# nemjit001/surf-path-tracer

Measured on AMD Instinct MI355X. Metric: Mrays/s at 1280×720, 256 spp, indoor scene; 1/2/4/8 MI355X + CPU ref, higher is better.
Workload: dtype f32; 1 GPU; C3; scene=bundled indoor (main.cpp:161-346), width=1280, height=720, spp=256, renders=7, step=one complete 256-frame render including its drain, bounces=unbounded + russian roulette, zero_cutoff=True, parallelism=single GPU

## Files before the change

surf-path-tracer_amd/csrc/device/types.h:

```cpp
#pragma once
#include <hip/hip_runtime.h>
#include <stdint.h>
#include "lds_layout.h"

namespace surfdev {

constexpr uint32_t kUnset = 0xffffffffu;
constexpr uint32_t kFlagMedium = 1u, kFlagSpecular = 2u;
constexpr int kBlock = 256;

struct DevInstance {
    float Minv[16];
    float M[16];
    uint32_t triOffset, idxOffset, nodeOffset, material;
    float area;
    uint32_t affineInv;
    uint32_t affine;
    uint32_t _pad;
};

struct DevMaterial {
    float emit, refl, refr, ior;
    float ec[4], albedo[4], absorb[4];
};

struct TraceInst {
    float4 m0, m1, m2, m3;
    uint4 meta;
    float4 r0, r1, r2, r3;
    float4 wlo, whi;
};
constexpr uint32_t kLdsTraceInst = 64;

struct DevScene {
    const TraceInst* tinst;
    const float4* nodes;
    const float4* tris;
    const float4* normals;
    const float4* verts;
    const float4* tlasNodes;
    const uint32_t* tlasIdx;
    const DevInstance* inst;
    const DevMaterial* mats;
    const uint2* lights;
    uint32_t nLights;
    uint32_t sbNode0, sbRecN, sbTri0, sbTriN;
    const float4* sbRec;
    uint32_t nInst, nMats;
    uint32_t tlasLeafCount;
    uint32_t finiteBoxes;
    uint32_t nodes4G;
    const float* wnodes;
    uint32_t nWnodes;
    uint32_t laneW;
    uint32_t bgType;
    float bgColor[3], bgA[3], bgB[3];
    float cellLo[3], cellScale[3];
    uint32_t nHeavy, keyMode;
    float4 hvLo[3], hvHi[3];
};

struct DevCamera {
    float pos[3], firstPixel[3], uVec[3], vVec[3], diskU[3], diskV[3];
    float invW, invH;
    uint32_t defocus;
};

struct Pool { float4* od; float4* T; uint8_t* key; };

constexpr uint32_t kShBins = 16;
#ifndef SURF_SH_XCDS
#define SURF_SH_XCDS 1
#endif
#ifndef SURF_SH_STRIDE
#define SURF_SH_STRIDE 32
#endif
constexpr uint32_t kShXcds = SURF_SH_XCDS, kShStride = SURF_SH_STRIDE;
constexpr uint32_t kShSegs = kShBins * kShXcds + 1u;
struct ShadowQ {
    float4* od; float4* c;
    uint32_t* cur;
    uint32_t region;
    uint32_t bins;
};

struct Counters {
    uint32_t nIn[2];
    uint32_t app[2];
    uint32_t maxSeg;
    uint32_t zeroCutoff;
    uint32_t segMax;
    uint32_t survN;
    uint32_t survCap;
    uint32_t rowNext;
    uint32_t permFrames, permA;
    uint32_t spp;
    unsigned long long issued[2];
    unsigned long long limit;
    unsigned long long baseFrame;
    unsigned long long ev[16];
    uint32_t capped[64];
    unsigned long long evS[32][16];
    unsigned long long dbg[8];
};
constexpr uint32_t kStripes = 32;
constexpr int kEvents = 9;

struct StreamGeom {
    const uint32_t* rows;
    uint32_t width, npx, window;
    const uint32_t* perm;
};

constexpr uint32_t kLeafTagC = 0x80000000u;
constexpr uint32_t kLeafTag = 0x80000000u;
constexpr uint32_t kLeafInW = 3;

constexpr uint32_t kLdsInst = 64, kLdsMats = 64, kLdsLights = 64;

constexpr int kDenoiseMaxIterations = 6;

static_assert(sizeof(TraceInst) == 4 * layout::kTraceInstWords && sizeof(DevInstance) == 4 * layout::kInstanceWords &&
                  sizeof(DevMaterial) == 4 * layout::kMaterialWords && sizeof(uint2) == 4 * layout::kLightWords &&
                  sizeof(float4) * 4 == 4 * layout::kNodeRecWords && sizeof(float4) * 3 == 4 * layout::kTriRecWords,
              "lds_layout.h states the table elements' sizes");

}
```

surf-path-tracer_amd/csrc/device/wavefront_kernels.h:

```cpp
#pragma once
#include <hip/hip_runtime.h>
#include <type_traits>
#include "surf_math.h"
#include "types.h"

namespace surfdev {

#ifndef SURF_SHADE_WAVES
#define SURF_SHADE_WAVES 4
#endif
#ifndef SURF_SEG_TIMING
#define SURF_SEG_TIMING 0
#endif
#ifndef SURF_TAIL_WAVES
#define SURF_TAIL_WAVES 3
#endif
#ifndef SURF_TRACE_WAVES
#define SURF_TRACE_WAVES 2
#endif
#ifndef SURF_TRACE_WAVES_EXT
#define SURF_TRACE_WAVES_EXT 6
#endif
#ifndef SURF_COOP_WAVES
#define SURF_COOP_WAVES 4
// ... 268 lines not shown
                    } else {
                        float eL, eR;
                        wBoxes<FIN>(rc, o, rd, depth, eL, eR);
                        bool g;
                        if (ANY) g = eL == kFarAway;
                        else g = eL > eR;
                        const float en = g ? eR : eL, ef = g ? eL : eR;
                        if (en == kFarAway) {
                            if (df == kFarAway) goto pop;
                            ref = refF;
                            continue;
                        }
                        if (df != kFarAway) { *sp = refF; sp += stride; }
                        const uint32_t pN = f2u(g ? rc.d.w : rc.d.z), pF = f2u(g ? rc.d.z : rc.d.w);
                        if (ef != kFarAway) { *sp = pF ? pF : nodeOff + lC + (g ? 0u : 1u); sp += stride; }
                        ref = pN ? pN : nodeOff + lC + (g ? 1u : 0u);
                        continue;
                    }
                }
            }
        }
        if (leafTest<ANY>(tri, lf, cnt, o, d, depth, hu, hv, hprim)) {
            if (ANY) return true;
            any = true;
        }
    pop:
        if (sp == bottom) break;
        sp -= stride;
        ref = *sp;
    }
    return any;
}

__device__ __forceinline__ float rowDot(float4 r, float x, float y, float z, float w) {
    const float a = r.x * x + r.y * y;
    const float b = r.z * z + r.w * w;
    return a + b;
}

__device__ __forceinline__ void instanceRay(const TraceInst& I, V3 o, V3 d, V3& oo, V3& dd) {
    oo = mk3(rowDot(I.m0, o.x, o.y, o.z, 1.0f), rowDot(I.m1, o.x, o.y, o.z, 1.0f), rowDot(I.m2, o.x, o.y, o.z, 1.0f));
    if (!I.meta.z) oo = divs(oo, rowDot(I.m3, o.x, o.y, o.z, 1.0f));
    dd = mk3(rowDot(I.m0, d.x, d.y, d.z, 0.0f), rowDot(I.m1, d.x, d.y, d.z, 0.0f), rowDot(I.m2, d.x, d.y, d.z, 0.0f));
}

template <bool ANY, bool LW = false, bool STG = false, typename SK = uint32_t>
__device__ __forceinline__ bool instanceTrace(const DevScene& S, const TraceInst& I, V3 o, V3 d, float& depth, float& hu,
                                              float& hv, uint32_t& hprim, SK* stk, uint32_t stride, uint32_t base,
                                              const float4* sN = nullptr) {
    V3 oo, dd;
    instanceRay(I, o, d, oo, dd);
    if (f2u(I.r1.w) != 0u)
        return leafTestUniform<ANY>(S.tris + 3u * I.meta.y, f2u(I.r0.w), f2u(I.r1.w), oo, dd, depth, hu, hv, hprim);
    const V3 rd = mk3(1.0f / dd.x, 1.0f / dd.y, 1.0f / dd.z);
    const bool fin = S.finiteBoxes && finite3(oo) && finite3(rd);
    if constexpr (LW)
        return fin ? blasTraceW<ANY, true>(S, I, oo, dd, rd, depth, hu, hv, hprim, stk, stride, base)
                   : blasTraceW<ANY, false>(S, I, oo, dd, rd, depth, hu, hv, hprim, stk, stride, base);
    if (fin) return blasTrace<ANY, true, STG, SK>(S, I, oo, dd, rd, depth, hu, hv, hprim, stk, stride, base, sN);
    return blasTrace<ANY, false, STG, SK>(S, I, oo, dd, rd, depth, hu, hv, hprim, stk, stride, base, sN);
}

struct TraceTables {
    const TraceInst* inst;
    const uint32_t* order;
};

__device__ __forceinline__ TraceTables stageTrace(const DevScene& S, uint32_t* lds, uint32_t at) {
    TraceInst* tab = reinterpret_cast<TraceInst*>(lds + at);
    uint32_t* order = reinterpret_cast<uint32_t*>(tab + S.nInst);
    const uint32_t n16 = S.nInst * (uint32_t)(sizeof(TraceInst) / 16);
    for (uint32_t k = threadIdx.x; k < n16; k += blockDim.x) reinterpret_cast<float4*>(tab)[k] = reinterpret_cast<const float4*>(S.tinst)[k];
    for (uint32_t k = threadIdx.x; k < S.nInst; k += blockDim.x) order[k] = S.tlasIdx[k];
    __syncthreads();
    return TraceTables{tab, order};
}

template <bool LDS_INST>
__device__ __forceinline__ TraceTables traceTables(const DevScene& S, uint32_t* lds, uint32_t at) {
    if (LDS_INST) return stageTrace(S, lds, at);
    return TraceTables{S.tinst, S.tlasIdx};
}

template <bool ANY, bool LW = false, bool STG = false, typename SK = uint32_t>
__device__ __forceinline__ bool traceScene(const DevScene& S, const TraceTables& Tt, V3 o, V3 d, float& depth, float& hu, float& hv,
                                           uint32_t& hinst, uint32_t& hprim, SK* stk, uint32_t stride, const float4* sN = nullptr) {
    bool any = false;
    if (S.tlasLeafCount) {
        const V3 rdw = mk3(1.0f / d.x, 1.0f / d.y, 1.0f / d.z);
        const bool cullOk = finite3(o) && finite3(rdw);
        for (uint32_t k = 0; k < S.tlasLeafCount; ++k) {
            const uint32_t ii = Tt.order[k];
            const TraceInst& I = Tt.inst[ii];
            if (cullOk && I.wlo.w != 0.0f) {
                const float tx0 = (I.wlo.x - o.x) * rdw.x, tx1 = (I.whi.x - o.x) * rdw.x;
                const float ty0 = (I.wlo.y - o.y) * rdw.y, ty1 = (I.whi.y - o.y) * rdw.y;
                const float tz0 = (I.wlo.z - o.z) * rdw.z, tz1 = (I.whi.z - o.z) * rdw.z;
                const float t0 = fmaxf(fmaxf(fminf(tx0, tx1), fminf(ty0, ty1)), fminf(tz0, tz1));
                const float t1 = fminf(fminf(fmaxf(tx0, tx1), fmaxf(ty0, ty1)), fmaxf(tz0, tz1));
                if (t1 < t0 || t1 < 0.0f || t0 >= depth) continue;
            }
            const bool hitI = (STG && !LW && I.meta.x == S.sbNode0 && I.meta.y == S.sbTri0)
                                  ? instanceTrace<ANY, false, true, SK>(S, I, o, d, depth, hu, hv, hprim, stk, stride, 0u, sN)
                                  : instanceTrace<ANY, LW, false, SK>(S, I, o, d, depth, hu, hv, hprim, stk, stride, 0u);
            if (hitI) {
                if (ANY) return true;
                any = true;
                hinst = ii;
            }
        }
        return any;
    }
    const V3 rd = mk3(1.0f / d.x, 1.0f / d.y, 1.0f / d.z);
    uint32_t sp = 0, node = 0;
    for (;;) {
        const float4* nd = S.tlasNodes + 4u * node;
        float4 q0 = nd[0], q1 = nd[1], q2 = nd[2], q3 = nd[3];
        pin(q0); pin(q1); pin(q2); pin(q3);
        const uint32_t lf = f2u(q0.w), cnt = f2u(q1.w);
        if (cnt != 0u) {
            for (uint32_t k = 0; k < cnt; ++k) {
                const uint32_t ii = Tt.order[lf + k];
                if (instanceTrace<ANY, LW, false, SK>(S, Tt.inst[ii], o, d, depth, hu, hv, hprim, stk, stride, sp)) {
                    if (ANY) return true;
                    any = true;
                    hinst = ii;
                }
            }
            if (sp == 0) break;
            node = stk[(--sp) * stride];
            continue;
        }
        float dn = slab(q0.x, q0.y, q0.z, q1.x, q1.y, q1.z, o, rd, depth);
        float df = slab(q2.x, q2.y, q2.z, q3.x, q3.y, q3.z, o, rd, depth);
        uint32_t cn = lf, cf = lf + 1u;
        if (dn > df) { const float t = dn; dn = df; df = t; const uint32_t c = cn; cn = cf; cf = c; }
        if (dn == kFarAway) {
            if (sp == 0) break;
            node = stk[(--sp) * stride];
        } else {
            node = cn;
            if (df != kFarAway) stk[(sp++) * stride] = cf;
        }
    }
    return any;
}

template <int CTRL>
__device__ __forceinline__ float dppMov(float v) {
    return __int_as_float(__builtin_amdgcn_mov_dpp(__float_as_int(v), CTRL, 0xF, 0xF, false));
}
constexpr int kDppSwap1 = 0xB1;
constexpr int kDppShr2 = 0x112, kDppShr4 = 0x114;

__device__ __forceinline__ uint32_t planeDword(uint32_t l) {
    if (l < 12u) return (l / 6u) * 8u + (l & 1u) * 4u + ((l % 6u) >> 1);
    return l == 12u ? 3u : (l == 13u ? 7u : 0u);
}
__device__ __forceinline__ float pick3(V3 v, uint32_t a) { return a == 0u ? v.x : (a == 1u ? v.y : v.z); }

__device__ __forceinline__ void slabPair(float v, float oA, float rdA, float depth, float& d0, float& d1) {
    const float t = (v - oA) * rdA;
    const float tp = dppMov<kDppSwap1>(t);
    const float t0a = tmin(t, tp), t1a = tmax(t, tp);
    const float t0x = dppMov<kDppShr4>(t0a), t0y = dppMov<kDppShr2>(t0a);
    const float t1x = dppMov<kDppShr4>(t1a), t1y = dppMov<kDppShr2>(t1a);
    const float m0 = tmax(tmax(t0x, t0y), t0a);
    const float m1 = tmin(tmin(t1x, t1y), t1a);
    const float dist = (m1 >= m0 && m0 < depth && m1 > 0.0f) ? m0 : kFarAway;
    d0 = __int_as_float(__builtin_amdgcn_readlane(__float_as_int(dist), 4));
    d1 = __int_as_float(__builtin_amdgcn_readlane(__float_as_int(dist), 10));
}

template <bool ANY>
// ... 2181 lines not shown
```

surf-path-tracer_amd/csrc/host/scene_upload.hip:

```cpp
#include "host/surf_ctx.h"

#include <algorithm>
#include <cfloat>
#include <cmath>
#include <cstdlib>
#include <cstring>

#include "device/surf_math.h"

namespace {

struct TreeWalk {
    uint32_t depth = 0;
    bool ok = true;
    std::string why;
};

TreeWalk walkTree(const surf_bvh_node* nodes, uint32_t nodeCount, uint32_t offset, uint32_t idxCount, uint32_t idxOffset,
                  std::vector<float4>& out, std::vector<uint8_t>& leafSeen, std::vector<uint32_t>* owner = nullptr) {
    TreeWalk w;
    std::vector<std::pair<uint32_t, uint32_t>> st{{0u, 0u}};
    size_t visits = 0;
    while (!st.empty()) {
        auto [local, dep] = st.back();
        st.pop_back();
        if (++visits > (size_t)nodeCount + 1 || dep > 4096) { w.ok = false; w.why = "BVH has a cycle"; return w; }
        const uint64_t g = (uint64_t)offset + local;
        if (g >= nodeCount) { w.ok = false; w.why = "BVH node index out of range"; return w; }
        const surf_bvh_node& n = nodes[g];
        float4* rec = &out[4 * g];
        if (owner) (*owner)[g] = offset;
        rec[0].w = u2f(n.left_first);
        rec[1].w = u2f(n.count);
        if (n.count != 0) {
            if ((uint64_t)idxOffset + n.left_first + n.count > idxCount) { w.ok = false; w.why = "BVH leaf range out of range"; return w; }
            for (uint32_t k = 0; k < n.count; ++k) leafSeen[idxOffset + n.left_first + k] = 1;
            w.depth = std::max(w.depth, dep);
            continue;
        }
        const uint64_t l = (uint64_t)offset + n.left_first;
        if (l + 1 >= nodeCount) { w.ok = false; w.why = "BVH child index out of range"; return w; }
        const surf_bvh_node& L = nodes[l];
        const surf_bvh_node& R = nodes[l + 1];
        rec[0] = make_float4(L.bb_min.x, L.bb_min.y, L.bb_min.z, rec[0].w);
        rec[1] = make_float4(L.bb_max.x, L.bb_max.y, L.bb_max.z, rec[1].w);
        rec[2] = make_float4(R.bb_min.x, R.bb_min.y, R.bb_min.z, 0.0f);
        rec[3] = make_float4(R.bb_max.x, R.bb_max.y, R.bb_max.z, 0.0f);
        st.push_back({n.left_first + 1, dep + 1});
        st.push_back({n.left_first, dep + 1});
    }
    return w;
}

constexpr uint64_t kLdsLightBlas = 20480;

struct InstanceTables {
    std::vector<DevInstance> inst;
    std::vector<TraceInst> tinst;
    std::vector<float4> tnodes;
    std::vector<uint32_t> tidx;
    std::vector<uint2> lights;
    uint32_t tlasDepth = 0, tlasLeafCount = 0;
    uint32_t nHeavy = 0;
    float4 hvLo[3], hvHi[3];
    uint32_t hvInst[3] = {0, 0, 0};
};

void setKeys(surf_ctx* c, DevScene& S, const InstanceTables& T) {
    c->heavyInst.assign(T.hvInst, T.hvInst + T.nHeavy);
    c->permValid = false;
    c->aovValid = false;
    S.nHeavy = T.nHeavy;
    for (uint32_t h = 0; h < 3; ++h) {
        S.hvLo[h] = h < T.nHeavy ? T.hvLo[h] : make_float4(0, 0, 0, 0);
        S.hvHi[h] = h < T.nHeavy ? T.hvHi[h] : make_float4(0, 0, 0, 0);
    }
    S.keyMode = T.nHeavy ? c->keyMode : 0u;
    S.sbNode0 = S.sbRecN = S.sbTri0 = S.sbTriN = 0u;
    S.sbRec = nullptr;
    if (c->ldsLightBlas && !T.lights.empty()) {
        bool one = true;
        const DevInstance* L0 = T.lights[0].x < T.inst.size() ? &T.inst[T.lights[0].x] : nullptr;
        for (const uint2& L : T.lights)
            one = one && L0 && L.x < T.inst.size() && T.inst[L.x].nodeOffset == L0->nodeOffset &&
                  T.inst[L.x].idxOffset == L0->idxOffset && T.inst[L.x].triOffset == L0->triOffset;
        const auto sb = one ? c->stagedBlas.find(L0->nodeOffset) : c->stagedBlas.end();
        const bool small = c->nBlasNodes < 65536u && T.tnodes.size() / 4 < 65536u;
        if (small && sb != c->stagedBlas.end() && sb->second.tri0 == L0->idxOffset) {
            S.sbNode0 = sb->first; S.sbRec = sb->second.rec; S.sbRecN = sb->second.recN;
            S.sbTri0 = sb->second.tri0; S.sbTriN = sb->second.triN;
        }
    }
}

int buildInstanceTables(surf_ctx* c, const surf_gpu_instance* instances, uint32_t n, const uint32_t* tlasIdx,
                        const surf_bvh_node* tlasNodes, uint32_t nTlas, const surf_light* lights, uint32_t nLights, InstanceTables& T) {
    auto affine = [](const float* m) { return m[3] == 0.0f && m[7] == 0.0f && m[11] == 0.0f && m[15] == 1.0f; };
    T.inst.resize(n);
    T.tinst.resize(n);
    for (uint32_t i = 0; i < n; ++i) {
        const surf_gpu_instance& g = instances[i];
        const auto root = c->blasRoots.find(std::make_tuple(g.bvh_node_offset, g.bvh_idx_offset, g.tri_offset));
        if (root == c->blasRoots.end() || g.material_offset >= c->nMaterials)
            return fail(c, SURF_ERR_INVALID, "instance " + std::to_string(i) + ": offsets do not name an uploaded BLAS/material");
        DevInstance& D = T.inst[i];
        std::memcpy(D.Minv, g.inv_transform, sizeof D.Minv);
        std::memcpy(D.M, g.transform, sizeof D.M);
        D.triOffset = g.tri_offset; D.idxOffset = g.bvh_idx_offset; D.nodeOffset = g.bvh_node_offset; D.material = g.material_offset;
        D.area = g.area;
        D.affineInv = affine(g.inv_transform) ? 1u : 0u;
        D.affine = affine(g.transform) ? 1u : 0u;
        const float* m = D.Minv;
        TraceInst& R = T.tinst[i];
        R.m0 = make_float4(m[0], m[4], m[8], m[12]);
        R.m1 = make_float4(m[1], m[5], m[9], m[13]);
        R.m2 = make_float4(m[2], m[6], m[10], m[14]);
        R.m3 = make_float4(m[3], m[7], m[11], m[15]);
        R.meta = make_uint4(D.nodeOffset, D.idxOffset, D.affineInv, i);
        R.r0 = root->second[0]; R.r1 = root->second[1]; R.r2 = root->second[2]; R.r3 = root->second[3];
        R.wlo = make_float4(0, 0, 0, 0);
        R.whi = make_float4(0, 0, 0, 0);
        const auto bb = c->blasBounds.find(g.tri_offset);
        double A[3][3], t[3], B[3][3];
        for (int r = 0; r < 3; ++r) {
            for (int q = 0; q < 3; ++q) A[r][q] = (double)g.inv_transform[4 * q + r];
            t[r] = (double)g.inv_transform[12 + r];
        }
        const double det = A[0][0] * (A[1][1] * A[2][2] - A[1][2] * A[2][1]) - A[0][1] * (A[1][0] * A[2][2] - A[1][2] * A[2][0]) +
                           A[0][2] * (A[1][0] * A[2][1] - A[1][1] * A[2][0]);
        if (bb != c->blasBounds.end() && D.affineInv && std::isfinite(det) && det != 0.0) {
            B[0][0] = (A[1][1] * A[2][2] - A[1][2] * A[2][1]) / det; B[0][1] = (A[0][2] * A[2][1] - A[0][1] * A[2][2]) / det;
            B[0][2] = (A[0][1] * A[1][2] - A[0][2] * A[1][1]) / det; B[1][0] = (A[1][2] * A[2][0] - A[1][0] * A[2][2]) / det;
            B[1][1] = (A[0][0] * A[2][2] - A[0][2] * A[2][0]) / det; B[1][2] = (A[0][2] * A[1][0] - A[0][0] * A[1][2]) / det;
            B[2][0] = (A[1][0] * A[2][1] - A[1][1] * A[2][0]) / det; B[2][1] = (A[0][1] * A[2][0] - A[0][0] * A[2][1]) / det;
            B[2][2] = (A[0][0] * A[1][1] - A[0][1] * A[1][0]) / det;
            double na = 0.0, nb = 0.0;
            for (int r = 0; r < 3; ++r)
                for (int q = 0; q < 3; ++q) { na += A[r][q] * A[r][q]; nb += B[r][q] * B[r][q]; }
            const double cond = std::sqrt(na * nb);
            double lo[3] = {HUGE_VAL, HUGE_VAL, HUGE_VAL}, hi[3] = {-HUGE_VAL, -HUGE_VAL, -HUGE_VAL};
            for (int corner = 0; corner < 8; ++corner) {
                const double p[3] = {bb->second[(corner & 1) ? 3 : 0] - t[0], bb->second[(corner & 2) ? 4 : 1] - t[1],
                                     bb->second[(corner & 4) ? 5 : 2] - t[2]};
                for (int r = 0; r < 3; ++r) {
                    const double w = B[r][0] * p[0] + B[r][1] * p[1] + B[r][2] * p[2];
                    lo[r] = std::min(lo[r], w); hi[r] = std::max(hi[r], w);
                }
            }
            double mag = 0.0;
            for (int r = 0; r < 3; ++r) mag = std::max({mag, std::fabs(lo[r]), std::fabs(hi[r]), hi[r] - lo[r]});
            const double pad = 1e-4 * mag * std::max(1.0, cond) + 1e-6;
            bool ok = std::isfinite(mag) && mag < 1e30;
            float flo[3], fhi[3];
            for (int r = 0; r < 3; ++r) {
                flo[r] = (float)(lo[r] - pad); fhi[r] = (float)(hi[r] + pad);
                ok = ok && std::isfinite(flo[r]) && std::isfinite(fhi[r]);
            }
            if (ok) {
                R.wlo = make_float4(flo[0], flo[1], flo[2], 1.0f);
                R.whi = make_float4(fhi[0], fhi[1], fhi[2], 0.0f);
            }
        }
    }
    T.tnodes.assign((size_t)nTlas * 4, make_float4(0, 0, 0, 0));
    std::vector<uint8_t> tseen(n, 0);
    TreeWalk tw = walkTree(tlasNodes, nTlas, 0, n, 0, T.tnodes, tseen);
    if (!tw.ok) return fail(c, SURF_ERR_INVALID, "TLAS: " + tw.why);
    T.tlasDepth = tw.depth;
    T.tidx.assign(tlasIdx, tlasIdx + n);
    for (uint32_t v : T.tidx) if (v >= n) return fail(c, SURF_ERR_INVALID, "TLAS index out of range");
    T.tlasLeafCount = tlasNodes[0].count;
    if (T.tlasLeafCount && tlasNodes[0].left_first != 0) T.tlasLeafCount = 0;
    if (T.tlasLeafCount) {
        std::vector<std::pair<uint32_t, uint32_t>> big;
        for (uint32_t i = 0; i < n; ++i) {
            const auto it = c->blasSlots.find(instances[i].tri_offset);
            const uint32_t tris = it == c->blasSlots.end() ? 0u : it->second;
            if (tris >= 64 && T.tinst[i].wlo.w != 0.0f) big.push_back({tris, i});
        }
        std::stable_sort(big.begin(), big.end(), [](const auto& a, const auto& b) { return a.first > b.first; });
        for (size_t h = 0; h < big.size() && h < 3; ++h) {
            T.hvLo[h] = T.tinst[big[h].second].wlo;
            T.hvHi[h] = T.tinst[big[h].second].whi;
            T.hvInst[h] = big[h].second;
            T.nHeavy = (uint32_t)h + 1;
        }
    }
    T.lights.resize(nLights);
    for (uint32_t l = 0; l < nLights; ++l) {
        const surf_light& L = lights[l];
        if (L.light_instance_idx >= n || L.primitive_count == 0 ||
            (uint64_t)instances[L.light_instance_idx].tri_offset + L.primitive_count > c->nTriangles)
            return fail(c, SURF_ERR_INVALID, "light " + std::to_string(l) + " out of range");
        T.lights[l] = make_uint2(L.light_instance_idx, L.primitive_count);
    }
    return SURF_OK;
}


struct BlasWalk {
    std::vector<float4> nodes;
    std::vector<int64_t> idxTri;
    std::vector<uint32_t> owner;
    uint32_t maxDepth = 0;
};
int walkBlases(surf_ctx* c, const surf_scene_desc* d, BlasWalk& B) {
    B.idxTri.assign(d->blas_index_count, -1);
    B.nodes.assign((size_t)d->blas_node_count * 4, make_float4(0, 0, 0, 0));
    B.owner.assign(d->blas_node_count, kUnset);
    std::vector<uint8_t> walked(d->blas_node_count, 0);
    for (uint32_t i = 0; i < d->instance_count; ++i) {
        const surf_gpu_instance& g = d->instances[i];
        if (g.tri_offset >= d->triangle_count || g.material_offset >= d->material_count ||
            g.bvh_node_offset >= d->blas_node_count || g.bvh_idx_offset >= d->blas_index_count)
            return fail(c, SURF_ERR_INVALID, "instance " + std::to_string(i) + " offsets out of range");
        if (walked[g.bvh_node_offset]) continue;
        std::vector<uint8_t> leaf(d->blas_index_count, 0);
        TreeWalk w = walkTree(d->blas_nodes, d->blas_node_count, g.bvh_node_offset, d->blas_index_count, g.bvh_idx_offset, B.nodes, leaf,
                              &B.owner);
        if (!w.ok) return fail(c, SURF_ERR_INVALID, "instance " + std::to_string(i) + ": " + w.why);
        B.maxDepth = std::max(B.maxDepth, w.depth);
        walked[g.bvh_node_offset] = 1;
        for (uint32_t k = 0; k < d->blas_index_count; ++k)
            if (leaf[k]) {
                if (B.idxTri[k] >= 0 && B.idxTri[k] != (int64_t)g.tri_offset) return fail(c, SURF_ERR_INVALID, "BLAS index range shared by two meshes");
                B.idxTri[k] = g.tri_offset;
            }
    }
    return SURF_OK;
}

struct CompactBlas { std::vector<float4> recs; uint32_t tri0, triN; };
std::map<uint32_t, CompactBlas> compactBlases(const surf_scene_desc* d, const std::vector<float4>& nodes) {
    std::map<uint32_t, CompactBlas> compact;
    for (uint32_t i = 0; i < d->instance_count; ++i) {
        const uint32_t root = d->instances[i].bvh_node_offset;
        if (compact.count(root) || d->blas_nodes[root].count != 0) continue;
        std::vector<float4> recs;
        std::vector<uint32_t> order{root};
        uint32_t slots = 0;
        bool ok = true;
        for (size_t k = 0; k < order.size() && ok; ++k) {
            const uint32_t g = order[k];
            const float4* r = &nodes[4 * (size_t)g];
            uint32_t ref[2];
            for (int ch = 0; ch < 2; ++ch) {
                const uint32_t cg = root + f2u(r[0].w) + (uint32_t)ch;
                const surf_bvh_node& q = d->blas_nodes[cg];
                if (q.count != 0) {
                    ok = ok && q.count < 32768u && q.left_first < 65536u;
                    ref[ch] = kLeafTagC | (q.count << 16) | (q.left_first & 0xffffu);
                    slots = std::max(slots, q.left_first + q.count);
                } else {
                    ok = ok && order.size() < 32768u;
                    ref[ch] = (uint32_t)order.size();
                    order.push_back(cg);
                }
            }
            recs.push_back(make_float4(r[0].x, r[0].y, r[0].z, u2f(ref[0])));
            recs.push_back(make_float4(r[1].x, r[1].y, r[1].z, u2f(ref[1])));
            recs.push_back(make_float4(r[2].x, r[2].y, r[2].z, 0.0f));
            recs.push_back(make_float4(r[3].x, r[3].y, r[3].z, 0.0f));
            ok = ok && (recs.size() / 4) * 64 + (uint64_t)slots * 48 <= kLdsLightBlas;
        }
        if (ok) compact[root] = CompactBlas{std::move(recs), d->instances[i].bvh_idx_offset, slots};
    }
    return compact;
}

struct TriangleRecords {
// ... 240 lines not shown
```

surf-path-tracer_amd/csrc/host/surf_ctx.h:

```cpp
#pragma once
#include <hip/hip_runtime.h>

#include <array>
#include <cstdio>
#include <map>
#include <string>
#include <tuple>
#include <vector>

#include "surf_hip.h"
#include "device/types.h"

using namespace surfdev;

constexpr uint32_t kMaxStack = 120;

struct surf_ctx {
    int device = 0;
    hipStream_t stream = nullptr;
    uint32_t width = 0, height = 0;
    std::vector<uint32_t> rows;
    uint32_t npx = 0;
    uint32_t capacity = 0;
    uint32_t window = 0;
    bool windowFixed = false;
    bool profiling = false;
    std::string err;

    bool hasScene = false;
    uint32_t extBlock = 128;
    bool connectGlobal = false;
    bool extStack16 = true;
    bool regenCount = true;
    bool ldsTables = false;
    DevScene S{};
    std::vector<void*> sceneAllocs;
    uint32_t stackDepth = 0;
    uint32_t nInstances = 0, nTriangles = 0, nBlasNodes = 0;
    uint32_t nMaterials = 0, nLightsUp = 0, tlasNodeCount = 0, maxBlasDepth = 0;
    std::map<std::tuple<uint32_t, uint32_t, uint32_t>, std::array<float4, 4>> blasRoots;
    std::map<uint32_t, std::array<double, 6>> blasBounds;
    std::map<uint32_t, uint32_t> blasSlots;
    bool reorder = true;
    bool permValid = false;
    uint32_t* dPerm = nullptr;
    void* aov[SURF_AOV_COUNT] = {};
    bool aovValid = false;
    float aovKernelMs = 0.0f;
    float4* dn[4] = {};
    size_t dnCap = 0;
    float4* dnIn[4] = {};
    size_t dnInCap = 0;
    hipEvent_t dnEv[kDenoiseMaxIterations + 2] = {};
    float dnMs[kDenoiseMaxIterations + 1] = {};
    uint32_t dnLdsMax = 2;
    float4* tp[7] = {};
    size_t tpCap = 0;
    int tpCur = 0;
    bool tpHave = false;
    surf_camera_ubo tpCam{};
    std::vector<surf_gpu_instance> tpInst;
    float4* tpIn[9] = {};
    size_t tpInCap = 0;
    float* tpMotion = nullptr;
    uint32_t tpMotionCap = 0;
    std::vector<float> tpMotionHost;
    hipEvent_t tpEv[2] = {};
    float tpMs = 0.0f;
    float4* sv[3] = {};
    size_t svCap = 0;
    int svCur = 0;
    bool svHave = false;
    float4* svIn[4] = {};
    size_t svInCap = 0;
    hipEvent_t svEv[kDenoiseMaxIterations + 3] = {};
    float svMs[kDenoiseMaxIterations + 2] = {};
    bool svVarStaged = true;
    float4* ff[1] = {};
    size_t ffCap = 0;
    float4* ffIn[2] = {};
    size_t ffInCap = 0;
    hipEvent_t ffEv[2] = {};
    float ffMs = 0.0f;
    std::vector<surf_gpu_instance> instHost;
    bool loopLag = true;
    size_t extLdsPad = 0, conLdsPad = 0;
    bool ldsLightBlas = true;
    struct StagedBlas { const float4* rec; uint32_t recN, tri0, triN; };
    std::map<uint32_t, StagedBlas> stagedBlas;
    uint32_t permA = 0, permFrames = 0;
    std::vector<uint32_t> heavyInst;
    uint32_t keyMode = 2;
    bool hasCamera = false;
    DevCamera cam{};
    surf_camera_ubo camUbo{};

    bool allocated = false;
    Pool pool[2]{};
    float4* hitTUV = nullptr;
    uint32_t* hitInst = nullptr;
    ShadowQ Q{};
    float4* rad = nullptr;
    float4* acc = nullptr;
    uint32_t* dRows = nullptr;
    Counters* ctr = nullptr;
    Counters* hctr = nullptr;
    uint32_t* frameDone = nullptr;
    struct Snap { Counters* h = nullptr; uint32_t* fd = nullptr; uint64_t acc = 0, open = 0; int phases = 0; hipEvent_t ev = nullptr; };
    static constexpr int kSnaps = 2;
    Snap snap[kSnaps];
    int snapHead = 0, snapCount = 0;
    uint64_t issuePerPhase = 0;
    bool pipeline = true;
    static constexpr uint32_t kLimitRing = 16;
    uint64_t* hLimit = nullptr;
    uint32_t hLimitNext = 0;
    hipEvent_t tev[2][2] = {};
    bool tevPending[2] = {false, false};
    int tevCur = 0;
    uint32_t* dOutRGBA = nullptr;
    std::vector<void*> wfAllocs;
    uint64_t totalSamples = 0;

    bool streamActive = false;
    uint64_t baseFrame = 0;
    uint64_t targetFrames = 0;
    uint64_t accPasses = 0;
    uint32_t spp = 1;
    uint32_t streamMaxSeg = 0;
    int zeroCutoff = -1;
    uint64_t pushedLimit = 0;
    uint32_t tailPaths = 0;
    uint32_t tailBudget = 16;
    Pool surv[2]{};
    uint32_t survCap = 0;
    uint32_t coopMax = 0;
    uint32_t coopAll = 150000;
    int drainReplays = 1;
    bool drainShort = false;
    bool regenFirst = false;
    int traceMode = 0;
    bool connectStaged = false;
    bool tailPair = true;
    uint32_t cus = 256;
    bool sortRays = true;
    bool sortPool = true;
    bool sortShadow = true;
    uint32_t* order = nullptr;
    uint32_t* binHist = nullptr;
    bool overlap = true;
    hipStream_t side = nullptr;
    std::vector<hipEvent_t> capEv;
    uint32_t tailLanes = 0;
    uint32_t segMaxBase = 0;
    uint64_t tailFirstRays = 0;

    hipGraphExec_t graphExec = nullptr, graphExecShort = nullptr;
    hipGraph_t graph = nullptr, graphShort = nullptr;
    uint32_t gridWork = 0, gridRegen = 0, gridExtend = 0, gridConnect = 0;

    hipEvent_t ev0 = nullptr, ev1 = nullptr;
    std::vector<hipEvent_t> pev;
    uint32_t* hPhaseN = nullptr;
    FILE* phaseLog = nullptr;
    surf_stats stats{};
    unsigned long long evBase[kEvents] = {};
};

namespace surfhost {
void setGlobalError(const std::string& e);
int endStream(surf_ctx* c);
void destroyGraph(surf_ctx* c);
int drainStream(surf_ctx* c);
int featurePlanes(surf_ctx* c);
int growImages(surf_ctx* c, float4** planes, int count, size_t& cap, size_t npx);
// ... 53 lines not shown
```

surf-path-tracer_amd/csrc/surf_hip.hip:

```cpp
#include "host/surf_ctx.h"

#include <algorithm>
#include <chrono>
#include <cmath>
#include <cstdlib>
#include <cstring>
#include <mutex>

#include "device/wavefront_kernels.h"
#include "device/denoise_kernels.h"

namespace {

#ifndef SURF_PHASES_GRAPH
#define SURF_PHASES_GRAPH 16
#endif
constexpr int kPhasesPerGraph = SURF_PHASES_GRAPH;
static_assert(kPhasesPerGraph % 2 == 0, "even: parity returns to 0 after a replay");
#ifndef SURF_PHASES_SHORT
#define SURF_PHASES_SHORT 4
#endif
constexpr int kPhasesShort = SURF_PHASES_SHORT;
static_assert(kPhasesShort % 2 == 0 && kPhasesShort <= kPhasesPerGraph, "even: parity returns to 0 after a replay");
constexpr int kPhaseEvents = 6;
// ... 814 lines not shown
        int rc = buildGraph(c);
        if (rc) return rc;
    }
    SURF_CHECK(c, hipEventRecord(c->ev0, c->stream));
    int rc = pump(c, true, 0);
    if (rc) return rc;
    SURF_CHECK(c, hipEventRecord(c->ev1, c->stream));
    SURF_CHECK(c, hipEventSynchronize(c->ev1));
    float ms = 0;
    (void)hipEventElapsedTime(&ms, c->ev0, c->ev1);
    c->stats.ms_total += ms;
    return SURF_OK;
}

}

int surfhost::drainStream(surf_ctx* c) { return ensureDrained(c); }
int surfhost::featurePlanes(surf_ctx* c) { return ensureAov(c); }
int surfhost::growImages(surf_ctx* c, float4** planes, int count, size_t& cap, size_t npx) { return growPlanes(c, planes, count, cap, npx); }
int surfhost::denoisePlanes(surf_ctx* c, uint32_t w, uint32_t h, const float4* acc, const float4* pos, const float4* nrm,
                            const float4* alb, const surf_denoise_params& P, const float4** result) {
    return runDenoise(c, w, h, acc, pos, nrm, alb, P, result);
}
const char* surfhost::denoiseParamsError(const surf_denoise_params* p) { return denoiseParamError(p); }

int surfhost::endStream(surf_ctx* c) {
    int rc = ensureDrained(c);
    if (rc) return rc;
    if (c->streamActive) {
        unsigned long long e[kEvents];
        streamEvents(*c->hctr, e);
        for (int k = 0; k < kEvents; ++k) c->evBase[k] += e[k];
        c->segMaxBase = std::max(c->segMaxBase, c->hctr->segMax);
    }
    c->streamActive = false;
    return SURF_OK;
}

namespace {

std::vector<uint32_t> shardRows(uint32_t height, uint32_t shard, uint32_t shards, uint32_t block) {
    std::vector<uint32_t> rows;
    if (block == 0) {
        const uint32_t r0 = (uint32_t)((uint64_t)height * shard / shards), r1 = (uint32_t)((uint64_t)height * (shard + 1) / shards);
        for (uint32_t r = r0; r < r1; ++r) rows.push_back(r);
    } else {
        for (uint32_t r = 0; r < height; ++r)
            if ((r / block) % shards == shard) rows.push_back(r);
    }
    return rows;
}

int createCtx(int dev, uint32_t w, uint32_t h, std::vector<uint32_t> rows, surf_ctx** out) {
    if (!out) return fail(nullptr, SURF_ERR_INVALID, "out is NULL");
    *out = nullptr;
    if (w == 0 || h == 0 || rows.empty()) return fail(nullptr, SURF_ERR_INVALID, "empty frame or shard");
    if ((uint64_t)w * rows.size() > (1ull << 31)) return fail(nullptr, SURF_ERR_INVALID, "shard too large");
    int count = 0;
    if (hipGetDeviceCount(&count) != hipSuccess || dev < 0 || dev >= count) return fail(nullptr, SURF_ERR_NO_DEVICE, "no HIP device " + std::to_string(dev));
    hipDeviceProp_t prop;
    if (hipGetDeviceProperties(&prop, dev) != hipSuccess) return fail(nullptr, SURF_ERR_NO_DEVICE, "hipGetDeviceProperties failed");
    if (std::string(prop.gcnArchName).find("gfx950") == std::string::npos)
        return fail(nullptr, SURF_ERR_NO_DEVICE, std::string("device is ") + prop.gcnArchName + ", this build targets gfx950");
    uint32_t extBlock = 128;
    if (const char* e = std::getenv("SURF_EXTEND_BLOCK")) {
        const int b = std::atoi(e);
        if (b != 128 && b != 256) return fail(nullptr, SURF_ERR_INVALID, std::string("SURF_EXTEND_BLOCK must be 128 or 256, not ") + e);
        extBlock = (uint32_t)b;
    }
    auto* c = new surf_ctx();
    c->capEv.assign(2 * kPhasesPerGraph, nullptr);
    c->pev.assign(kPhasesPerGraph * kPhaseEvents + 1, nullptr);
    c->device = dev;
    c->extBlock = extBlock;
    if (const char* e = std::getenv("SURF_SORT")) {
        c->sortRays = e[0] != '0';
        c->sortPool = e[0] != '3';
        c->sortShadow = e[0] != '2';
    }
    if (const char* e = std::getenv("SURF_CONNECT_GLOBAL")) c->connectGlobal = e[0] != '0';
    if (const char* e = std::getenv("SURF_EXT_STACK16")) c->extStack16 = e[0] != '0';
    if (const char* e = std::getenv("SURF_REGEN_COUNT")) c->regenCount = e[0] != '0';
    if (const char* e = std::getenv("SURF_KEY")) c->keyMode = e[0] == '0' ? 0u : (e[0] == '1' ? 1u : 2u);
    if (const char* e = std::getenv("SURF_OVERLAP")) c->overlap = e[0] != '0';
    if (const char* e = std::getenv("SURF_LOOP_LAG")) c->loopLag = e[0] != '0';
    if (const char* e = std::getenv("SURF_EXT_LDS_PAD")) c->extLdsPad = (size_t)std::max(0, std::atoi(e));
    if (const char* e = std::getenv("SURF_CON_LDS_PAD")) c->conLdsPad = (size_t)std::max(0, std::atoi(e));
    if (const char* e = std::getenv("SURF_LDS_LIGHTBLAS")) c->ldsLightBlas = e[0] != '0';
    if (const char* e = std::getenv("SURF_REORDER")) c->reorder = e[0] != '0';
    if (const char* e = std::getenv("SURF_TAIL_PAIR")) c->tailPair = e[0] != '0';
    if (const char* e = std::getenv("SURF_DRAIN_SHORT")) c->drainShort = e[0] == '1';
    if (const char* e = std::getenv("SURF_REGEN_FIRST")) c->regenFirst = e[0] == '1';
    if (const char* e = std::getenv("SURF_PIPELINE")) c->pipeline = e[0] != '0';
    if (const char* e = std::getenv("SURF_DENOISE_LDS")) c->dnLdsMax = (uint32_t)std::max(0, std::atoi(e));
    if (const char* e = std::getenv("SURF_SVGF_LDS")) c->svVarStaged = std::atoi(e) != 0;
    c->width = w;
    c->height = h;
    c->rows = std::move(rows);
    c->npx = (uint32_t)(w * c->rows.size());
    if (hipSetDevice(dev) != hipSuccess || hipStreamCreateWithFlags(&c->stream, hipStreamNonBlocking) != hipSuccess ||
        hipEventCreate(&c->ev0) != hipSuccess || hipEventCreate(&c->ev1) != hipSuccess ||
        hipStreamCreateWithFlags(&c->side, hipStreamNonBlocking) != hipSuccess) {
        delete c;
        return fail(nullptr, SURF_ERR_HIP, "stream/event creation failed");
    }
    for (auto& e : c->capEv)
        if (hipEventCreateWithFlags(&e, hipEventDisableTiming) != hipSuccess) {
            delete c;
            return fail(nullptr, SURF_ERR_HIP, "event creation failed");
        }
    if (hipMalloc(&c->acc, (size_t)c->npx * sizeof(float4)) != hipSuccess ||
        hipMalloc(&c->dRows, c->rows.size() * sizeof(uint32_t)) != hipSuccess) {
        surf_destroy(c);
        return fail(nullptr, SURF_ERR_OOM, "accumulator allocation failed");
    }
    (void)hipMemset(c->acc, 0, (size_t)c->npx * sizeof(float4));
    (void)hipMemcpy(c->dRows, c->rows.data(), c->rows.size() * sizeof(uint32_t), hipMemcpyHostToDevice);
    *out = c;
    return SURF_OK;
}

}

extern "C" {

int surf_abi_version(void) { return SURF_ABI_VERSION; }

int surf_device_count(int* count) {
    if (!count) return SURF_ERR_INVALID;
    *count = 0;
    if (hipGetDeviceCount(count) != hipSuccess) { *count = 0; return fail(nullptr, SURF_ERR_NO_DEVICE, "hipGetDeviceCount failed"); }
    return SURF_OK;
}

int surf_create(int dev, uint32_t w, uint32_t h, uint32_t r0, uint32_t r1, surf_ctx** out) {
    if (r0 >= r1 || r1 > h) return fail(nullptr, SURF_ERR_INVALID, "row range out of frame");
    std::vector<uint32_t> rows;
    for (uint32_t r = r0; r < r1; ++r) rows.push_back(r);
    return createCtx(dev, w, h, std::move(rows), out);
}

int surf_create_sharded(int dev, uint32_t w, uint32_t h, uint32_t shard, uint32_t shards, uint32_t block, surf_ctx** out) {
    if (shards == 0 || shard >= shards) return fail(nullptr, SURF_ERR_INVALID, "bad shard index");
    return createCtx(dev, w, h, shardRows(h, shard, shards, block), out);
}

void surf_destroy(surf_ctx* c) {
    if (!c) return;
    (void)hipSetDevice(c->device);
    if (c->stream) (void)hipStreamSynchronize(c->stream);
    destroyGraph(c);
    freeList(c->sceneAllocs);
    freeList(c->wfAllocs);
    if (c->hctr) (void)hipHostFree(c->hctr);
    if (c->hLimit) (void)hipHostFree(c->hLimit);
    for (auto& sn : c->snap) {
        if (sn.h) (void)hipHostFree(sn.h);
        if (sn.fd) (void)hipHostFree(sn.fd);
        if (sn.ev) (void)hipEventDestroy(sn.ev);
    }
    for (auto& pr : c->tev)
        for (auto& e : pr) if (e) (void)hipEventDestroy(e);
    if (c->rad) (void)hipFree(c->rad);
    if (c->frameDone) (void)hipFree(c->frameDone);
    for (auto& e : c->pev) if (e) (void)hipEventDestroy(e);
    if (c->hPhaseN) (void)hipHostFree(c->hPhaseN);
// ... 512 lines not shown
```

Baseline: 519.1 Mrays/s.

## Batch consecutive TLAS leaves sharing a tiny triangle range into one run

On the host, finds runs of consecutive top-level leaves whose instances reference the same small triangle range (one or two triangles), and marks them with head and member bitmasks in the scene. In traceScene, such a run is handled by leafRun: it first box-culls every instance in the run into a bitmask, then tests the shared triangles once per surviving instance without going through the generic instance BVH traversal. The aim is to cut per-instance traversal setup and reloads of the same triangle data for repeated small instances. It costs extra bitmask checks in the hot TLAS loop, more code in the trace kernel (possible register pressure), and only applies when the scene has at most 64 leaves.

```diff
diff --git a/surf-path-tracer_amd/csrc/device/types.h b/surf-path-tracer_amd/csrc/device/types.h
--- a/surf-path-tracer_amd/csrc/device/types.h
+++ b/surf-path-tracer_amd/csrc/device/types.h
@@ -58,7 +58,9 @@
     float cellLo[3], cellScale[3];
     uint32_t nHeavy, keyMode;
     float4 hvLo[3], hvHi[3];
+    unsigned long long runHead, runMember;
 };
+constexpr uint32_t kLeafRunTris = 2, kLeafRunMin = 2, kLeafRunMax = 32, kLeafRunPositions = 63;
 
 struct DevCamera {
     float pos[3], firstPixel[3], uVec[3], vVec[3], diskU[3], diskV[3];
diff --git a/surf-path-tracer_amd/csrc/device/wavefront_kernels.h b/surf-path-tracer_amd/csrc/device/wavefront_kernels.h
--- a/surf-path-tracer_amd/csrc/device/wavefront_kernels.h
+++ b/surf-path-tracer_amd/csrc/device/wavefront_kernels.h
@@ -374,6 +374,47 @@
     return TraceTables{S.tinst, S.tlasIdx};
 }
 
+template <bool ANY>
+__device__ __forceinline__ bool leafRun(const DevScene& S, const TraceTables& Tt, uint32_t k0, unsigned long long more, V3 o, V3 d,
+                                        V3 rdw, bool cullOk, float& depth, float& hu, float& hv, uint32_t& hinst, uint32_t& hprim) {
+    uint32_t m = 0u, n = 0u;
+    do {
+        const TraceInst& I = Tt.inst[Tt.order[k0 + n]];
+        bool take = true;
+        if (cullOk && I.wlo.w != 0.0f) {
+            const float tx0 = (I.wlo.x - o.x) * rdw.x, tx1 = (I.whi.x - o.x) * rdw.x;
+            const float ty0 = (I.wlo.y - o.y) * rdw.y, ty1 = (I.whi.y - o.y) * rdw.y;
+            const float tz0 = (I.wlo.z - o.z) * rdw.z, tz1 = (I.whi.z - o.z) * rdw.z;
+            const float t0 = fmaxf(fmaxf(fminf(tx0, tx1), fminf(ty0, ty1)), fminf(tz0, tz1));
+            const float t1 = fminf(fminf(fmaxf(tx0, tx1), fmaxf(ty0, ty1)), fmaxf(tz0, tz1));
+            take = !(t1 < t0 || t1 < 0.0f || t0 >= depth);
+        }
+        m |= take ? 1u << n : 0u;
+        ++n;
+    } while ((more >> (k0 + n)) & 1ull);
+    const TraceInst& H = Tt.inst[Tt.order[k0]];
+    const float4* tri = S.tris + 3u * (H.meta.y + f2u(H.r0.w));
+    const uint32_t cnt = f2u(H.r1.w);
+    bool any = false;
+    while (m) {
+        const uint32_t ii = Tt.order[k0 + (uint32_t)__ffs((int)m) - 1u];
+        m &= m - 1u;
+        const TraceInst& I = Tt.inst[ii];
+        const V3 oo = mk3(rowDot(I.m0, o.x, o.y, o.z, 1.0f), rowDot(I.m1, o.x, o.y, o.z, 1.0f), rowDot(I.m2, o.x, o.y, o.z, 1.0f));
+        const V3 dd = mk3(rowDot(I.m0, d.x, d.y, d.z, 0.0f), rowDot(I.m1, d.x, d.y, d.z, 0.0f), rowDot(I.m2, d.x, d.y, d.z, 0.0f));
+        for (uint32_t t = 0; t < cnt; ++t) {
+            const float4 a = tri[3u * t], b = tri[3u * t + 1u], c = tri[3u * t + 2u];
+            float u, v;
+            if (triHit(xyz(a), xyz(b), xyz(c), oo, dd, depth, u, v)) {
+                if (ANY) return true;
+                any = true;
+                hu = u; hv = v; hprim = f2u(a.w); hinst = ii;
+            }
+        }
+    }
+    return any;
+}
+
 template <bool ANY, bool LW = false, bool STG = false, typename SK = uint32_t>
 __device__ __forceinline__ bool traceScene(const DevScene& S, const TraceTables& Tt, V3 o, V3 d, float& depth, float& hu, float& hv,
                                            uint32_t& hinst, uint32_t& hprim, SK* stk, uint32_t stride, const float4* sN = nullptr) {
@@ -381,7 +422,16 @@
     if (S.tlasLeafCount) {
         const V3 rdw = mk3(1.0f / d.x, 1.0f / d.y, 1.0f / d.z);
         const bool cullOk = finite3(o) && finite3(rdw);
+        const unsigned long long runMore = S.runMember & ~S.runHead;
         for (uint32_t k = 0; k < S.tlasLeafCount; ++k) {
+            if (__builtin_expect((S.runMember >> k) & 1ull, 0)) {
+                if ((runMore >> k) & 1ull) continue;
+                if (leafRun<ANY>(S, Tt, k, runMore, o, d, rdw, cullOk, depth, hu, hv, hinst, hprim)) {
+                    if (ANY) return true;
+                    any = true;
+                }
+                continue;
+            }
             const uint32_t ii = Tt.order[k];
             const TraceInst& I = Tt.inst[ii];
             if (cullOk && I.wlo.w != 0.0f) {
diff --git a/surf-path-tracer_amd/csrc/host/scene_upload.hip b/surf-path-tracer_amd/csrc/host/scene_upload.hip
--- a/surf-path-tracer_amd/csrc/host/scene_upload.hip
+++ b/surf-path-tracer_amd/csrc/host/scene_upload.hip
@@ -64,6 +64,7 @@
     uint32_t nHeavy = 0;
     float4 hvLo[3], hvHi[3];
     uint32_t hvInst[3] = {0, 0, 0};
+    unsigned long long runHead = 0, runMember = 0;
 };
 
 void setKeys(surf_ctx* c, DevScene& S, const InstanceTables& T) {
@@ -76,6 +77,8 @@
         S.hvHi[h] = h < T.nHeavy ? T.hvHi[h] : make_float4(0, 0, 0, 0);
     }
     S.keyMode = T.nHeavy ? c->keyMode : 0u;
+    S.runHead = c->leafRun ? T.runHead : 0ull;
+    S.runMember = c->leafRun ? T.runMember : 0ull;
     S.sbNode0 = S.sbRecN = S.sbTri0 = S.sbTriN = 0u;
     S.sbRec = nullptr;
     if (c->ldsLightBlas && !T.lights.empty()) {
@@ -186,6 +189,27 @@
             T.nHeavy = (uint32_t)h + 1;
         }
     }
+    if (T.tlasLeafCount && T.tlasLeafCount <= 64u) {
+        auto runLeaf = [&](uint32_t k) {
+            const TraceInst& R = T.tinst[T.tidx[k]];
+            return R.meta.z != 0u && f2u(R.r1.w) >= 1u && f2u(R.r1.w) <= kLeafRunTris;
+        };
+        auto sameRange = [&](uint32_t k, uint32_t j) {
+            const TraceInst &A = T.tinst[T.tidx[k]], &B = T.tinst[T.tidx[j]];
+            return A.meta.y == B.meta.y && f2u(A.r0.w) == f2u(B.r0.w) && f2u(A.r1.w) == f2u(B.r1.w);
+        };
+        const uint32_t end = std::min(T.tlasLeafCount, kLeafRunPositions);
+        for (uint32_t k = 0; k < end;) {
+            uint32_t len = 0;
+            if (runLeaf(k))
+                for (len = 1; k + len < end && len < kLeafRunMax && runLeaf(k + len) && sameRange(k, k + len);) ++len;
+            if (len >= kLeafRunMin) {
+                T.runHead |= 1ull << k;
+                for (uint32_t j = 0; j < len; ++j) T.runMember |= 1ull << (k + j);
+            }
+            k += std::max(len, 1u);
+        }
+    }
     T.lights.resize(nLights);
     for (uint32_t l = 0; l < nLights; ++l) {
         const surf_light& L = lights[l];
diff --git a/surf-path-tracer_amd/csrc/host/surf_ctx.h b/surf-path-tracer_amd/csrc/host/surf_ctx.h
--- a/surf-path-tracer_amd/csrc/host/surf_ctx.h
+++ b/surf-path-tracer_amd/csrc/host/surf_ctx.h
@@ -91,6 +91,7 @@
     uint32_t permA = 0, permFrames = 0;
     std::vector<uint32_t> heavyInst;
     uint32_t keyMode = 2;
+    bool leafRun = true;
     bool hasCamera = false;
     DevCamera cam{};
     surf_camera_ubo camUbo{};
diff --git a/surf-path-tracer_amd/csrc/surf_hip.hip b/surf-path-tracer_amd/csrc/surf_hip.hip
--- a/surf-path-tracer_amd/csrc/surf_hip.hip
+++ b/surf-path-tracer_amd/csrc/surf_hip.hip
@@ -920,6 +920,7 @@
     if (const char* e = std::getenv("SURF_EXT_STACK16")) c->extStack16 = e[0] != '0';
     if (const char* e = std::getenv("SURF_REGEN_COUNT")) c->regenCount = e[0] != '0';
     if (const char* e = std::getenv("SURF_KEY")) c->keyMode = e[0] == '0' ? 0u : (e[0] == '1' ? 1u : 2u);
+    if (const char* e = std::getenv("SURF_LEAF_RUN")) c->leafRun = e[0] != '0';
     if (const char* e = std::getenv("SURF_OVERLAP")) c->overlap = e[0] != '0';
     if (const char* e = std::getenv("SURF_LOOP_LAG")) c->loopLag = e[0] != '0';
     if (const char* e = std::getenv("SURF_EXT_LDS_PAD")) c->extLdsPad = (size_t)std::max(0, std::atoi(e));
```

Result: faster. 528.7 Mrays/s (median of 6 runs) (+1.9%).
